# samuel-watson/glmmrMCML

Hardware: AMD Instinct MI355X
Metric: MCML iters/sec x m chains (simlik evals/sec) (higher is better)
Workload: dtype f64

## Files before the change

### glmmrmcml_amd/csrc/debug_hooks.hip

```cpp
#include "dgemm_mfma.h"
#include "dgemm_dl.h"
#include "dgemm_band.h"

using namespace mcml;

extern "C" int glmmr_mcml_dbg_dgemm(int M, int N, int K, const double* A, int lda,
                                    const double* B, int ldb, int b_nmajor,
                                    double alpha, double beta, double* C, int ldc,
                                    int lower_only, int force_tile)
{
    int ndev = 0;
    if (hipGetDeviceCount(&ndev) != hipSuccess || ndev == 0) {
        set_error("no HIP device: libglmmr_mcml_hip has no CPU fallback");
        return MCML_ENODEVICE;
    }
    hipStream_t s = nullptr;
    DevMat dA, dB, dC;
    if (force_tile == 40) {
        MCML_REQUIRE(!b_nmajor && !lower_only, "dbg_dgemm: the direct-to-LDS kernel takes a K-major B and all tiles");
        const int kpad = round_up(K, 32);
        MCML_TRY(dA.alloc(M, K, 32));
        MCML_HIP(hipMemset(dA.d(), 0, sizeof(double) * (size_t)dA.ld * dA.cols_alloc));
        MCML_HIP(hipMemcpy2D(dA.d(), sizeof(double) * dA.ld, A, sizeof(double) * lda, sizeof(double) * M, K, hipMemcpyHostToDevice));
        MCML_TRY(dB.alloc(kpad, N));
// ... 20 lines not shown
                      : launch_gemm<false>(s, M, N, K, dA.d(), dA.ld, dB.d(), dB.ld, epi, lower_only != 0, force_tile);
    MCML_TRY(rc);
    MCML_TRY(download_matrix(C, ldc, dC.d(), dC.ld, M, N, s));
    return MCML_OK;
}

extern "C" int glmmr_mcml_dbg_dgemm_at(int M, int N, int K, const double* A, int lda, const double* B, int ldb,
                                       double alpha, double beta, double* C, int ldc, int force_tile)
{
    int ndev = 0;
    if (hipGetDeviceCount(&ndev) != hipSuccess || ndev == 0) {
        set_error("no HIP device: libglmmr_mcml_hip has no CPU fallback");
        return MCML_ENODEVICE;
    }
    MCML_REQUIRE(M > 0 && N > 0 && K > 0 && A && B && C, "dbg_dgemm_at: bad argument");
    const int K2 = round_up(K, 2);
    MCML_REQUIRE(lda >= K2 && ldb >= K2 && ldc >= M, "dbg_dgemm_at: a column of A and of B holds round_up(K, 2) = %d doubles", K2);
    hipStream_t s = nullptr;
    DevMat dA, dB, dC;
    MCML_TRY(upload_matrix(dA, A, K2, M, lda, s));
    MCML_TRY(upload_matrix(dB, B, K2, N, ldb, s));
    const bool inplace = C == B;
    MCML_REQUIRE(!inplace || (M == K && M <= 128 && ldc == ldb), "dbg_dgemm_at: in place needs M == K <= 128");
    if (!inplace) MCML_TRY(upload_matrix(dC, C, M, N, ldc, s));
    const DevMat& out = inplace ? dB : dC;
    EpiAxpby epi{out.d(), out.ld, alpha, beta};
    MCML_TRY(launch_gemm_at(s, M, N, K, dA.d(), dA.ld, dB.d(), dB.ld, epi, force_tile));
    MCML_TRY(download_matrix(C, ldc, out.d(), out.ld, M, N, s));
    return MCML_OK;
}

extern "C" int glmmr_mcml_dbg_dgemm_bench2(int M, int N, int K, int b_nmajor, int iters, int force_tile,
                                           int lower_only, double beta, double* ms_per_launch);
extern "C" int glmmr_mcml_dbg_dgemm_bench(int M, int N, int K, int b_nmajor, int iters,
                                          int force_tile, double* ms_per_launch)
{
    return glmmr_mcml_dbg_dgemm_bench2(M, N, K, b_nmajor, iters, force_tile, 0, 0.0, ms_per_launch);
}

extern "C" int glmmr_mcml_dbg_dgemm_bench2(int M, int N, int K, int b_nmajor, int iters, int force_tile,
                                           int lower_only, double beta, double* ms_per_launch)
{
    int ndev = 0;
    if (hipGetDeviceCount(&ndev) != hipSuccess || ndev == 0) {
        set_error("no HIP device: libglmmr_mcml_hip has no CPU fallback");
        return MCML_ENODEVICE;
    }
    hipStream_t s = nullptr;
    std::vector<double> hA((size_t)M * K), hB((size_t)K * N), hC((size_t)M * N, 0.0);
    uint64_t x = 88172645463325252ULL;
    auto rnd = [&]() { x ^= x << 13; x ^= x >> 7; x ^= x << 17; return (double)(x >> 11) / 9007199254740992.0 * 2 - 1; };
    for (auto& v : hA) v = rnd();
    for (auto& v : hB) v = rnd();
    DevMat dA, dB, dC;
    MCML_TRY(upload_matrix(dA, hA.data(), M, K, M, s));
    if (b_nmajor) MCML_TRY(upload_matrix(dB, hB.data(), N, K, N, s));
    else MCML_TRY(upload_matrix(dB, hB.data(), K, N, K, s));
    MCML_TRY(upload_matrix(dC, hC.data(), M, N, M, s));
    EpiAxpby epi{dC.d(), dC.ld, beta != 0.0 ? 1e-3 : 1.0, beta};
    const bool lo = lower_only != 0;
    auto go = [&]() {
        if (force_tile >= 20)
            return b_nmajor ? launch_gemm_dl<true>(s, M, N, K, dA.d(), dA.ld, dB.d(), dB.ld, epi, lo, force_tile - 19)
                            : launch_gemm_dl<false>(s, M, N, K, dA.d(), dA.ld, dB.d(), dB.ld, epi, lo, force_tile - 19);
        return b_nmajor ? launch_gemm<true>(s, M, N, K, dA.d(), dA.ld, dB.d(), dB.ld, epi, lo, force_tile)
                        : launch_gemm<false>(s, M, N, K, dA.d(), dA.ld, dB.d(), dB.ld, epi, lo, force_tile);
    };
    for (int i = 0; i < 3; i++) MCML_TRY(go());
    hipEvent_t e0, e1;
    MCML_HIP(hipEventCreate(&e0));
    MCML_HIP(hipEventCreate(&e1));
    MCML_HIP(hipEventRecord(e0, s));
    for (int i = 0; i < iters; i++) MCML_TRY(go());
    MCML_HIP(hipEventRecord(e1, s));
    MCML_HIP(hipEventSynchronize(e1));
    float ms = 0;
    MCML_HIP(hipEventElapsedTime(&ms, e0, e1));
    *ms_per_launch = ms / iters;
    (void)hipEventDestroy(e0);
    (void)hipEventDestroy(e1);
    return MCML_OK;
}

extern "C" int glmmr_mcml_dbg_dgemm_band(int M, int N, int K, const double* A, int lda, const double* B, int ldb,
                                         double* C, int ldc, int* tiles_executed)
{
    int ndev = 0;
    if (hipGetDeviceCount(&ndev) != hipSuccess || ndev == 0) {
        set_error("no HIP device: libglmmr_mcml_hip has no CPU fallback");
        return MCML_ENODEVICE;
    }
    MCML_REQUIRE(M > 0 && N > 0 && K > 0 && A && B && C, "dbg_dgemm_band: bad argument");
    hipStream_t s = nullptr;
    DevMat dA, dB, dC;
    MCML_TRY(dA.alloc(M, K, 32));
    MCML_HIP(hipMemset(dA.d(), 0, sizeof(double) * (size_t)dA.ld * dA.cols_alloc));
    MCML_HIP(hipMemcpy2D(dA.d(), sizeof(double) * dA.ld, A, sizeof(double) * lda, sizeof(double) * M, K, hipMemcpyHostToDevice));
    MCML_TRY(dB.alloc(round_up(K, 32), N));
    MCML_HIP(hipMemset(dB.d(), 0, sizeof(double) * (size_t)dB.ld * N));
    MCML_HIP(hipMemcpy2D(dB.d(), sizeof(double) * dB.ld, B, sizeof(double) * ldb, sizeof(double) * K, N, hipMemcpyHostToDevice));
    MCML_TRY(dC.alloc(M, N));
    MCML_HIP(hipMemset(dC.d(), 0, sizeof(double) * (size_t)dC.ld * N));
    MCML_REQUIRE(dlds_applicable(M, N, K, dA.d(), dA.ld, dA.cols_alloc, dB.d(), dB.ld), "dbg_dgemm_band: contract");
    const int nbands = (M + BD_BM - 1) / BD_BM;
    DevBuf kr;
    MCML_TRY(kr.ensure(sizeof(int) * 2 * nbands));
    hipLaunchKernelGGL(k_band_ranges, dim3(nbands), dim3(256), 0, s, dA.d(), dA.ld, M, K, kr.as<int>());
    MCML_HIP(hipGetLastError());
    std::vector<int> hk(2 * nbands);
    MCML_HIP(hipMemcpy(hk.data(), kr.p, sizeof(int) * 2 * nbands, hipMemcpyDeviceToHost));
    BandPlan plan;
    plan.reset(M, K, hk);
    if (tiles_executed) *tiles_executed = (int)plan.tiles;
    EpiAxpby epi{dC.d(), dC.ld, 1.0, 0.0};
    MCML_TRY(launch_gemm_band(s, plan, N, dA.d(), dA.ld, dB.d(), dB.ld, epi));
    MCML_TRY(download_matrix(C, ldc, dC.d(), dC.ld, M, N, s));
    return MCML_OK;
}

extern "C" int glmmr_mcml_dbg_band_clocks(int M, int N, int iters, int mode, double* out3)
{
    int ndev = 0;
    if (hipGetDeviceCount(&ndev) != hipSuccess || ndev == 0) {
        set_error("no HIP device: libglmmr_mcml_hip has no CPU fallback");
        return MCML_ENODEVICE;
    }
    hipStream_t s = nullptr;
    if (getenv("GLMMR_MCML_DBG_STREAM")) MCML_HIP(hipStreamCreateWithFlags(&s, hipStreamNonBlocking));
    std::vector<double> hA((size_t)M * M, 0.0), hB((size_t)M * N);
    uint64_t x = 88172645463325252ULL;
    auto rnd = [&]() { x ^= x << 13; x ^= x >> 7; x ^= x << 17; return (double)(x >> 11) / 9007199254740992.0 * 2 - 1; };
    const bool cst = getenv("GLMMR_MCML_DBG_DATA") && !strcmp(getenv("GLMMR_MCML_DBG_DATA"), "const");
    const bool dec = getenv("GLMMR_MCML_DBG_DATA") && !strcmp(getenv("GLMMR_MCML_DBG_DATA"), "decay");
    for (int j = 0; j < M; ++j) for (int i = j; i < M; ++i) hA[i + (size_t)j * M] = cst ? 1.0 : dec ? rnd() * std::exp(-(double)(i - j) / 40.0) : rnd();
    for (auto& v : hB) v = cst ? 1.0 : rnd();
    DevMat dA, dB, dC;
    MCML_TRY(dA.alloc(M, M, 32));
    MCML_HIP(hipMemset(dA.d(), 0, sizeof(double) * (size_t)dA.ld * dA.cols_alloc));
    MCML_HIP(hipMemcpy2D(dA.d(), sizeof(double) * dA.ld, hA.data(), sizeof(double) * M, sizeof(double) * M, M, hipMemcpyHostToDevice));
    MCML_TRY(dB.alloc(round_up(M, 32), N));
    MCML_HIP(hipMemset(dB.d(), 0, sizeof(double) * (size_t)dB.ld * N));
    MCML_HIP(hipMemcpy2D(dB.d(), sizeof(double) * dB.ld, hB.data(), sizeof(double) * M, sizeof(double) * M, N, hipMemcpyHostToDevice));
    MCML_TRY(dC.alloc(M, N));
    const int nbands = (M + BD_BM - 1) / BD_BM;
    DevBuf kr, clk;
    MCML_TRY(kr.ensure(sizeof(int) * 2 * nbands));
    MCML_TRY(clk.ensure(16));
    MCML_HIP(hipMemset(clk.p, 0, 16));
    hipLaunchKernelGGL(k_band_ranges, dim3(nbands), dim3(256), 0, s, dA.d(), dA.ld, M, M, kr.as<int>());
    std::vector<int> hk(2 * nbands);
    MCML_HIP(hipMemcpy(hk.data(), kr.p, sizeof(int) * 2 * nbands, hipMemcpyDeviceToHost));
    BandPlan plan;
    plan.reset(M, M, hk);
    const double tiles = (double)plan.tiles;
    EpiAxpby epi{dC.d(), dC.ld, 1.0, 0.0};
    if (mode < 0) {
        for (int i = 0; i < 3; i++)
            MCML_TRY((launch_gemm_band<EpiAxpby, false>(s, plan, N, dA.d(), dA.ld, dB.d(), dB.ld, epi)));
        hipEvent_t f0, f1;
        MCML_HIP(hipEventCreate(&f0));
        MCML_HIP(hipEventCreate(&f1));
        MCML_HIP(hipEventRecord(f0, s));
        for (int i = 0; i < iters; i++)
            MCML_TRY((launch_gemm_band<EpiAxpby, false>(s, plan, N, dA.d(), dA.ld, dB.d(), dB.ld, epi)));
        MCML_HIP(hipEventRecord(f1, s));
        MCML_HIP(hipEventSynchronize(f1));
        float fms = 0;
        MCML_HIP(hipEventElapsedTime(&fms, f0, f1));
        out3[0] = fms / iters; out3[1] = 0;
        out3[2] = 2.0 * 80.0 * 32.0 * tiles * N / (fms / iters * 1e-3) / 1e12;
        (void)hipEventDestroy(f0);
        (void)hipEventDestroy(f1);
        return MCML_OK;
    }
    if (mode & 16) {
        BandPlanDev* d = nullptr;
        MCML_TRY(plan.device_plan((N + BD_BN - 1) / BD_BN, s, &d));
        const int nb = d->nwg * d->gn;
        DevBuf st;
        MCML_TRY(st.ensure(sizeof(unsigned long long) * (8 + 8 * (size_t)nb)));
        for (int rep = 0; rep < 3; ++rep) {
            MCML_HIP(hipMemset(st.p, 0, sizeof(unsigned long long) * (8 + 8 * (size_t)nb)));
            MCML_TRY((launch_gemm_band<EpiAxpby, true>(s, plan, N, dA.d(), dA.ld, dB.d(), dB.ld, epi, st.as<unsigned long long>(), mode)));
            MCML_HIP(hipDeviceSynchronize());
        }
        std::vector<unsigned long long> h(8 + 8 * (size_t)nb);
        MCML_HIP(hipMemcpy(h.data(), st.p, sizeof(unsigned long long) * h.size(), hipMemcpyDeviceToHost));
        unsigned long long t0 = ~0ULL;
        for (int w = 0; w < nb; ++w) if (h[8 + 8 * w] && h[8 + 8 * w] < t0) t0 = h[8 + 8 * w];
        double mx[5] = {0, 0, 0, 0, 0}, sm[5] = {0, 0, 0, 0, 0};
        for (int w = 0; w < nb; ++w)
            for (int i = 0; i < 5; ++i) { double v = (double)(h[8 + 8 * w + i] - t0) * 0.01; sm[i] += v; if (v > mx[i]) mx[i] = v; }
        printf("band stamps (us from the first workgroup's start; %d workgroups, mean / max):\n", nb);
        const char* nm[5] = {"start", "ring filled", "K loop done", "epilogue issued", "end"};
        for (int i = 0; i < 5; ++i) printf("  %-16s %7.2f / %7.2f\n", nm[i], sm[i] / nb, mx[i]);
        if (mode & 32) for (int w = 0; w < nb; ++w) {
            printf("  wg %3d:", w);
            for (int i = 0; i < 5; ++i) printf(" %7.2f", (double)(h[8 + 8 * w + i] - t0) * 0.01);
// ... 213 lines not shown
```

### glmmrmcml_amd/csrc/dgemm_band.h

```cpp
#pragma once
#include "dgemm_dlds.h"
#include "band_plan.h"

namespace mcml {

struct BandP {
    GemmP g;
    const BandItem* items;
    const int* wg_ptr;
    int nwg;
    double* part;
    int mode;
    unsigned long long* clocks;
};

static __global__ __launch_bounds__(256) void k_band_ranges(const double* A, int lda, int M, int K, int* krange)
{
    __shared__ int smin[256], smax[256];
    const int band = blockIdx.x, r0 = band * BD_BM;
    const int rows = (M - r0 < BD_BM) ? (M - r0) : BD_BM;
    int kmin = 1 << 30, kmax = -1;
    for (int k = threadIdx.x; k < K; k += 256) {
        const double* col = A + r0 + (size_t)k * lda;
        bool nz = false;
// ... 207 lines not shown
                const double* bs = reinterpret_cast<const double*>(lds + st * BD_STAGE_BYTES + BD_A_BYTES);
#pragma unroll
                for (int ks = 0; ks < BD_BK / 4; ++ks) {
                    const int kk = 4 * ks + lk;
                    double a[5];
#pragma unroll
                    for (int i = 0; i < 5; ++i) a[i] = as[kk * BD_BM + 16 * i + l15];
                    const double b = bs[((kk >> 1) * BD_BN + wave * 16 + l15) * 2 + (kk & 1)];
#pragma unroll
                    for (int i = 0; i < 5; ++i)
                        acc[i][0] = __builtin_amdgcn_mfma_f64_16x16x4f64(b, a[i], acc[i][0], 0, 0, 0);
                }
                wait_leave(issued - kt - 2);
                __builtin_amdgcn_s_barrier();
                st = st + 1; if (st >= BD_STAGES) st = 0;
            }
        } else if (DBG && nk > 0) {
            int issued = 0;
            if (!(mode & 1)) {
                for (; issued < BD_STAGES - 1 && issued < nk; ++issued) issue(issued);
                wait_leave(issued - 1);
            }
            __builtin_amdgcn_s_barrier();
            int st = 0;
            double a[5] = {1.0 + lane, 2.0, 3.0, 4.0, 5.0}, b = 0.5 + lane;
            for (int kt = 0; kt < nk; ++kt) {
                if (!(mode & 1) && issued < nk) {
                    int sn = st + BD_STAGES - 1; if (sn >= BD_STAGES) sn -= BD_STAGES;
                    issue(sn);
                    ++issued;
                }
                const double* as = reinterpret_cast<const double*>(lds + st * BD_STAGE_BYTES);
                const double* bs = reinterpret_cast<const double*>(lds + st * BD_STAGE_BYTES + BD_A_BYTES);
#pragma unroll
                for (int ks = 0; ks < BD_BK / 4; ++ks) {
                    const int kk = 4 * ks + lk;
                    if (!(mode & 4)) {
#pragma unroll
                        for (int i = 0; i < 5; ++i) a[i] = as[kk * BD_BM + 16 * i + l15];
                        b = bs[((kk >> 1) * BD_BN + wave * 16 + l15) * 2 + (kk & 1)];
                    }
#pragma unroll
                    for (int i = 0; i < 5; ++i)
                        acc[i][0] = __builtin_amdgcn_mfma_f64_16x16x4f64(b, a[i], acc[i][0], 0, 0, 0);
                }
                if (!(mode & 1)) wait_leave(issued - kt - 2);
                if (!(mode & 2)) __builtin_amdgcn_s_barrier();
                st = st + 1; if (st >= BD_STAGES) st = 0;
            }
        }
        if (first_item) stamp(2);
        ++it;
        pre = false;
        if (it < it1) {
            load_item(it);
            const int nkn = item.kt1 - item.kt0;
            if (mode == 0 && nk > 0 && nkn > 0) {
                issued = 0;
                for (; issued < BD_STAGES - 1 && issued < nkn; ++issued) issue(issued);
                pre = true;
            }
        }
        if (slot < 0) {
            epi(acc, e_m0, n0 + wave * 16, lane, p.M, p.N, band);
        } else {
            double* P = bp.part + ((size_t)slot * p.gn + bj) * BD_TILE_ELEMS + (size_t)wave * (20 * 64) + lane;
#pragma unroll
            for (int i = 0; i < 5; ++i)
#pragma unroll
                for (int r = 0; r < 4; ++r) P[(i * 4 + r) * 64] = acc[i][0][r];
        }
        if (first_item) { stamp(3); first_item = false; }
        if (!pre) __builtin_amdgcn_s_barrier();
    }
    if constexpr (DBG)
        if (stamps) { asm volatile("s_waitcnt vmcnt(0)" ::: "memory"); stamp(4); }
    if constexpr (DBG)
        if (bp.clocks && blockIdx.x == 0 && tid == 0) {
            atomicAdd(bp.clocks, __builtin_amdgcn_s_memtime() - t0c);
            atomicAdd(bp.clocks + 1, __builtin_amdgcn_s_memrealtime() - t0r);
        }
}

template <class Epi>
__global__ __launch_bounds__(128) void k_band_reduce(const BandRed* red, const double* part, int gn, int M, int N, Epi epi)
{
    const BandRed rd = red[blockIdx.x];
    const int bj = blockIdx.y;
    const int lane = threadIdx.x & 63, wave = blockIdx.z * 2 + (threadIdx.x >> 6);
    d4 acc[5][1];
#pragma unroll
    for (int i = 0; i < 5; ++i) acc[i][0] = d4{0.0, 0.0, 0.0, 0.0};
    const size_t pstride = (size_t)gn * BD_TILE_ELEMS;
    const double* P0 = part + ((size_t)rd.s0 * gn + bj) * BD_TILE_ELEMS + (size_t)wave * (20 * 64) + lane;
    for (int s = rd.s0; s < rd.s1; s += 4) {
        double v[4][20];
#pragma unroll
        for (int u = 0; u < 4; ++u) {
            const double* P = P0 + (size_t)(s - rd.s0 + (s + u < rd.s1 ? u : 0)) * pstride;
#pragma unroll
            for (int t = 0; t < 20; ++t) v[u][t] = P[t * 64];
        }
#pragma unroll
        for (int u = 0; u < 4; ++u)
            if (s + u < rd.s1) {
#pragma unroll
                for (int i = 0; i < 5; ++i)
#pragma unroll
                    for (int r = 0; r < 4; ++r) acc[i][0][r] += v[u][i * 4 + r];
            }
    }
    epi(acc, rd.band * BD_BM, bj * BD_BN + wave * 16, lane, M, N, rd.band);
}

template <class Epi, bool DBG = false>
static inline int launch_gemm_band(hipStream_t s, BandPlan& plan, int N, const double* A, int lda,
                                   const double* B, int ldb, const Epi& epi,
                                   unsigned long long* clocks = nullptr, int mode = 0)
{
    const int gn = (N + BD_BN - 1) / BD_BN;
    BandPlanDev* d = nullptr;
    MCML_TRY(plan.device_plan(gn, s, &d));
    BandP bp;
    bp.clocks = clocks;
    bp.mode = mode;
    bp.g = GemmP{plan.M, N, plan.K, A, lda, B, ldb, 0, gn, 0};
    bp.items = d->items.as<BandItem>();
    bp.wg_ptr = d->wg_ptr.as<int>();
    bp.nwg = d->nwg;
    bp.part = d->part.d();
    MCML_TRY(ensure_dynamic_lds(reinterpret_cast<const void*>(&dgemm_band_kernel<Epi, DBG>), (int)BD_LDS_BYTES));
    hipLaunchKernelGGL((dgemm_band_kernel<Epi, DBG>), dim3(d->nwg * gn), dim3(512), BD_LDS_BYTES, s, bp, epi);
    if (d->nred > 0)
        hipLaunchKernelGGL((k_band_reduce<Epi>), dim3(d->nred, gn, 4), dim3(128), 0, s, d->red.as<BandRed>(),
                           d->part.d(), gn, plan.M, N, epi);
    MCML_HIP(hipGetLastError());
    return MCML_OK;
}


}
```

### glmmrmcml_amd/csrc/hmc.hip

```cpp
#include <algorithm>
#include <atomic>
#include <chrono>
#include "../../include/glmmr_mcml_c.h"
#include "ctx.h"
#include "dgemm_mfma.h"
#include "dgemm_dlds.h"
#include "dgemm_band.h"
#include "dgemm_skinny.h"
#include "glm.h"
#include "reduce.h"
#include "rng.h"
#include "hmc_cm.h"
#include "hmc_traj.h"

namespace mcml {

struct ChainArrays {
    double *e, *ebar, *H, *lpcur, *K0;
    int *steps, *acc;
    uint32_t* gen;
    long long* leap;
};

static ChainArrays chain_arrays(const HmcState& h)
// ... 65 lines not shown
    const double* e; const int* steps; int s; double post; int mode;
    __device__ __forceinline__ void elem(int m, int n, double accv) const {
        int st = 0; double en = 0.0;
        if (mode == 1) { st = steps[n]; en = e[n]; if (s >= st) return; }
        const size_t off = m + (size_t)n * ld;
        const double x = Xs[off];
        double g = -1.0 * x;
        g = g + post * accv;
        if (mode != 1 || s + 1 >= st) G[off] = g;
        if (mode == 1) {
            double rr = R[off];
            rr = rr + (en / 2) * g;
            if (s + 1 < st) {
                rr = rr + (en / 2) * g;
                UP[off] = x + en * rr;
            }
            R[off] = rr;
        }
    }
    template <int TM, int TN>
    __device__ __forceinline__ void operator()(d4 (&acc)[TM][TN], int mB, int nB, int lane, int M, int N,
                                               int) const {
#pragma unroll
        for (int j = 0; j < TN; ++j) {
            int stv[4]; double env[4]; bool inN[4]; size_t cb[4];
#pragma unroll
            for (int r = 0; r < 4; ++r) {
                const int n = nB + 16 * j + (lane >> 4) + 4 * r;
                inN[r] = n < N;
                const int nn = inN[r] ? n : 0;
                stv[r] = mode == 1 ? steps[nn] : 0;
                env[r] = mode == 1 ? e[nn] : 0.0;
                cb[r] = (size_t)nn * ld;
            }
            double xv[TM][4], rv[TM][4];
#pragma unroll
            for (int i = 0; i < TM; ++i) {
                const int m = mB + 16 * i + (lane & 15);
                const int mm = m < M ? m : 0;
#pragma unroll
                for (int r = 0; r < 4; ++r) {
                    xv[i][r] = Xs[mm + cb[r]];
                    rv[i][r] = mode == 1 ? R[mm + cb[r]] : 0.0;
                }
            }
#pragma unroll
            for (int r = 0; r < 4; ++r) {
                const double en = env[r];
                const bool more = s + 1 < stv[r];
#pragma unroll
                for (int i = 0; i < TM; ++i) {
                    const double x = xv[i][r];
                    double g = -1.0 * x;
                    g = g + post * acc[i][j][r];
                    acc[i][j][r] = g;
                    double rr = rv[i][r];
                    rr = rr + (en / 2) * g;
                    const double rr2 = rr + (en / 2) * g;
                    rr = more ? rr2 : rr;
                    rv[i][r] = rr;
                    xv[i][r] = x + en * rr;
                }
            }
#pragma unroll
            for (int r = 0; r < 4; ++r) {
                const bool act = inN[r] && (mode != 1 || s < stv[r]);
                if (!act) continue;
                const bool more = s + 1 < stv[r];
#pragma unroll
                for (int i = 0; i < TM; ++i) {
                    const int m = mB + 16 * i + (lane & 15);
                    if (m >= M) continue;
                    const size_t off = m + cb[r];
                    if (mode != 1 || !more) G[off] = acc[i][j][r];
                    if (mode == 1) {
                        if (more) UP[off] = xv[i][r];
                        R[off] = rv[i][r];
                    }
                }
            }
        }
    }
};


__global__ __launch_bounds__(256) void k_blockdiag_LV(int Q, int ncols, const int* start, const double* L, int ldl,
                                                      const double* V, int ldv, double* U, int ldu)
{
    const int q = blockIdx.x * 256 + threadIdx.x;
    if (q >= Q) return;
    const int s0 = start[q];
    for (int c = blockIdx.y; c < ncols; c += gridDim.y) {
        const double* v = V + (size_t)c * ldv;
        double acc = 0.0;
        for (int t = s0; t <= q; ++t) acc += L[q + (size_t)t * ldl] * v[t];
        U[q + (size_t)c * ldu] = acc;
    }
}

__global__ __launch_bounds__(256) void k_hmc_init(double* V, int ld, int Q, ChainArrays ca, uint64_t seed,
                                                  uint32_t chain_offset, uint32_t iter_idx, const double* inj_init)
{
    const int c = blockIdx.x;
    const uint32_t gid = chain_offset + (uint32_t)c;
    for (int q = threadIdx.x; q < Q; q += 256)
        V[q + (size_t)c * ld] = inj_init ? inj_init[q + (size_t)c * Q]
                                         : rng_normal(seed, (uint32_t)q, gid, 0u, 16u * iter_idx + 0u);
    if (threadIdx.x == 0) {
        ca.e[c] = 0.001; ca.ebar[c] = 1.0; ca.H[c] = 0.0; ca.acc[c] = 0; ca.leap[c] = 0;
        ca.gen[c] = chain_minstd_seed(seed, gid, iter_idx);
        ca.steps[c] = 1;
    }
}

template <int FL>
__device__ __forceinline__ double chain_log_prob(const double* MU, int ldm, int n, const double* X, int ldx,
                                                 int Q, const double* y, double var_par, int flink_rt, int c,
                                                 double* sh)
{
    const int flink = FL ? FL : flink_rt;
    double ll = 0, lp = 0;
    for (int i0 = threadIdx.x; i0 < n; i0 += 1024) {
        double m4[4], y4[4];
#pragma unroll
        for (int u = 0; u < 4; ++u) {
            const int i = i0 + 256 * u;
            m4[u] = i < n ? MU[i + (size_t)c * ldm] : 0.0;
            y4[u] = i < n ? y[i] : 0.0;
        }
#pragma unroll
        for (int u = 0; u < 4; ++u)
            if (i0 + 256 * u < n) ll += glm_logpdf(y4[u], m4[u], var_par, flink);
    }
    for (int k0 = threadIdx.x; k0 < Q; k0 += 1024) {
        double x4[4];
#pragma unroll
        for (int u = 0; u < 4; ++u) { const int k = k0 + 256 * u; x4[u] = k < Q ? X[k + (size_t)c * ldx] : 0.0; }
#pragma unroll
        for (int u = 0; u < 4; ++u)
            if (k0 + 256 * u < Q) lp += glm_logpdf(x4[u], 0, 1, 7);
    }
    double a = block_sum(ll, sh);
    double b = block_sum(lp, sh);
    return a + b;
}

template <int FL>
__global__ __launch_bounds__(256) void k_hmc_lp0(const double* MU, int ldm, int n, const double* V, int ld, int Q,
                                                 const double* y, double var_par, int flink, double* lpcur)
{
    __shared__ double sh[4];
    double v = chain_log_prob<FL>(MU, ldm, n, V, ld, Q, y, var_par, flink, blockIdx.x, sh);
    if (threadIdx.x == 0) lpcur[blockIdx.x] = v;
}

__global__ __launch_bounds__(256) void k_hmc_propose(const double* V, const double* GRAD, double* R, double* UP,
                                                     int ld, int Q, ChainArrays ca, double lambda, int max_steps,
                                                     uint64_t seed, uint32_t chain_offset, uint32_t iter_idx,
                                                     int it, const double* inj_mom, int C)
{
    __shared__ double sh[4];
    const int c = blockIdx.x;
    const uint32_t gid = chain_offset + (uint32_t)c;
    const double e = ca.e[c];
    double ss = 0;
    for (int q = threadIdx.x; q < Q; q += 256) {
// ... 705 lines not shown
```

### include/glmmr_mcml_c.h

```cpp
#ifndef GLMMR_MCML_C_H
#define GLMMR_MCML_C_H
#include <stdint.h>

#ifdef __cplusplus
extern "C" {
#endif

#define GLMMR_MCML_OK            0
#define GLMMR_MCML_EINVAL       -1
#define GLMMR_MCML_EUNSUPPORTED -2
#define GLMMR_MCML_ENOTPD       -3
#define GLMMR_MCML_ESINGULAR    -4
#define GLMMR_MCML_EHIP         -5
#define GLMMR_MCML_ENODEVICE    -6
#define GLMMR_MCML_ENOMEM       -7

const char* glmmr_mcml_last_error(void);


typedef struct glmmr_mcml_problem {
    const int32_t* cov;
    int            cov_rows;
    const double*  data;
    int            data_len;
// ... 171 lines not shown
                     double* theta, double* sigma);
int glmmr_mcml_simlik(const glmmr_mcml_problem* prob, const double* u, int ucols, const double* start,
                      int nstart, int trace, const glmmr_mcml_ext* ext, double* beta, double* theta,
                      double* sigma);
int glmmr_mcml_optim_sparse(const glmmr_mcml_problem* prob, const int32_t* Ap, const int32_t* Ai, int nnz,
                            const double* u, int ucols, const double* start, int nstart, int trace,
                            int mcnr, const glmmr_mcml_ext* ext, double* beta, double* theta,
                            double* sigma,
                            int32_t* Lp, int32_t* Li, double* Lx, double* D, int lcap);
int glmmr_mcml_sparse_factor_nnz(const int32_t* cov, int cov_rows, const double* data, int data_len);
int glmmr_mcml_simlik_sparse(const glmmr_mcml_problem* prob, const int32_t* Ap, const int32_t* Ai, int nnz,
                             const double* u, int ucols, const double* start, int nstart, int trace,
                             const glmmr_mcml_ext* ext, double* beta, double* theta, double* sigma);
int glmmr_mcml_hess(const glmmr_mcml_problem* prob, const double* u, int ucols, const double* start,
                    int nstart, double tol, int trace, const glmmr_mcml_ext* ext, double* H);
int glmmr_mcml_hess_sparse(const glmmr_mcml_problem* prob, const int32_t* Ap, const int32_t* Ai, int nnz,
                           const double* u, int ucols, const double* start, int nstart, double tol,
                           int trace, const glmmr_mcml_ext* ext, double* H);
int glmmr_mcml_aic(const glmmr_mcml_problem* prob, const double* u, int ucols, const double* beta_par,
                   int nbeta, const double* cov_par, int ncov, const glmmr_mcml_ext* ext, double* out);

int glmmr_mcml_la(const glmmr_mcml_problem* prob, const double* start, int nstart, int usehess, double tol,
                  int verbose, int trace, int maxiter, const glmmr_mcml_ext* ext, double* beta, double* theta,
                  double* sigma, double* se, double* u);
int glmmr_mcml_la_nr(const glmmr_mcml_problem* prob, const double* start, int nstart, int usehess, double tol,
                     int verbose, int trace, int maxiter, const glmmr_mcml_ext* ext, double* beta, double* theta,
                     double* sigma, double* se, double* u);
int glmmr_mcml_ctx_la(glmmr_mcml_ctx* ctx, const double* start, int nstart, int nr, int usehess, double tol,
                      int verbose, int trace, int maxiter, const glmmr_mcml_ext* ext, double* beta, double* theta,
                      double* sigma, double* se, double* u, int* converged, int* iters);

int glmmr_mcml_mvn_ll(const int32_t* cov, int cov_rows, const double* data, int data_len,
                      const double* eff_range, int eff_len, const double* gamma, int ngamma,
                      const double* u, int Q, int m, double* out);

int glmmr_mcml_dbg_theta_log(glmmr_mcml_ctx* ctx, int enable, double* out, int cap_rows, int* nrows);
int glmmr_mcml_dbg_emulate_world(glmmr_mcml_ctx* ctx, int world, int mode);
int glmmr_mcml_dbg_leaf_profile(glmmr_mcml_ctx* ctx, unsigned long long* out10);
int glmmr_mcml_dbg_la_probe(glmmr_mcml_ctx* ctx, const double* start, int nstart, int kind, const double* v,
                            double var_par, const double* par, int npar, double* out, double* v_out,
                            double* beta_out, double* sigma_out);
int glmmr_mcml_dbg_dgemm(int M, int N, int K, const double* A, int lda, const double* B, int ldb,
                         int b_nmajor, double alpha, double beta, double* C, int ldc,
                         int lower_only, int force_tile );
int glmmr_mcml_dbg_dgemm_at(int M, int N, int K, const double* A, int lda, const double* B, int ldb, double alpha,
                            double beta, double* C, int ldc, int force_tile);
int glmmr_mcml_dbg_chol(glmmr_mcml_ctx* ctx, int n, double* A, int lda, int m, const double* B, int ldb, double* Xfwd,
                        double* Ytrans, double* Zpotrs, double* Linv);
int glmmr_mcml_dbg_mvn_workspace(glmmr_mcml_ctx* ctx, int cand, double* L, int ldl, double* X, int ldx, int* dims);
int glmmr_mcml_dbg_log_prob_grad(glmmr_mcml_ctx* ctx, const double* beta, double var_par, const double* V,
                                 int ncols, double* lp, double* G);
int glmmr_mcml_dbg_normals(uint64_t seed, uint32_t chain, uint32_t prop, uint32_t tag, int n, double* out);
int glmmr_mcml_dbg_minstd(uint32_t seed, int n, double* out);
typedef double (*glmmr_mcml_objective)(const double* x, int n, void* user);
int glmmr_mcml_dbg_bobyqa(glmmr_mcml_objective f, void* user, int n, const double* x0, const double* lower,
                          const double* upper, double rhobeg, double rhoend, int maxfun, double* x_out,
                          double* f_out, int* nfev_out);
int glmmr_mcml_dbg_bobyqa_npt(glmmr_mcml_objective f, void* user, int n, const double* x0, const double* lower,
                              const double* upper, double rhobeg, double rhoend, int maxfun, int npt, double* x_out,
                              double* f_out, int* nfev_out);
int glmmr_mcml_dbg_bobyqa_batch(glmmr_mcml_objective f, void* user, int n, const double* x0, const double* lower,
                                const double* upper, double rhobeg, double rhoend, int maxfun, int width,
                                double* x_out, double* f_out, int* nfev_out, int* rounds_out);
typedef int (*glmmr_mcml_batch_objective)(const double* X, int n, int k, double* F, void* user);
int glmmr_mcml_dbg_bobyqa_rounds(glmmr_mcml_batch_objective fb, void* user, int n, const double* x0, const double* lower,
                                 const double* upper, double rhobeg, double rhoend, int maxfun, int width,
                                 double* x_out, double* f_out, int* nfev_out, int* rounds_out);
typedef int (*glmmr_mcml_parts_objective)(const double* X, int n, int k, double* logdet, double* sumsq, int* status,
                                          void* user);
int glmmr_mcml_dbg_theta_scale_rounds(glmmr_mcml_parts_objective fb, void* user, int n, const int* exps, int dim, int m,
                                      int grouped, const double* x0, const double* lower, const double* upper,
                                      double rhobeg, double rhoend, int maxfun, int width, double* x_out, double* f_out,
                                      int* nfev_out, int* rounds_out, long long* factorised_out);
int glmmr_mcml_dbg_theta_round(glmmr_mcml_ctx* ctx, const double* thetas, int k, double* out);
int glmmr_mcml_dbg_copy_roundtrip(const double* in, long long ld_in, double* out, long long ld_out, long long rows, long long cols);
int glmmr_mcml_dbg_fd_hessian(glmmr_mcml_objective f, void* user, int n, const double* x, double ndeps,
                              int usebounds, const double* lower, const double* upper, double* H);
int glmmr_mcml_dbg_dgemm_bench(int M, int N, int K, int b_nmajor, int iters, int force_tile,
                               double* ms_per_launch);
int glmmr_mcml_dbg_dgemm_bench2(int M, int N, int K, int b_nmajor, int iters, int force_tile, int lower_only,
                                double beta, double* ms_per_launch);
int glmmr_mcml_dbg_dgemm_band(int M, int N, int K, const double* A, int lda, const double* B, int ldb, double* C,
                              int ldc, int* tiles_executed);
int glmmr_mcml_dbg_band_clocks(int M, int N, int iters, int mode, double* out3);

#ifdef __cplusplus
}
#endif
#endif
```

Measured before the change: 1161.

## Add warp-specialised feeder form of band DGEMM with dedicated DMA waves

Adds a new band GEMM kernel in which four waves only issue global-to-LDS DMA loads through a multi-stage buffer. The other four waves only run f64 MFMA work on a 32-column slice each, with double-buffered LDS register reads. It is enabled by default, overridable through an env var, for the axpby and HMC forward/backward epilogues. The aim is to keep load issue and waitcnt stalls off the MFMA waves. The cost is half the waves doing no math and larger per-wave accumulators.

New measurement: 1223 (median of 6 runs). 5.3% higher.

```diff
diff --git a/glmmrmcml_amd/csrc/debug_hooks.hip b/glmmrmcml_amd/csrc/debug_hooks.hip
--- a/glmmrmcml_amd/csrc/debug_hooks.hip
+++ b/glmmrmcml_amd/csrc/debug_hooks.hip
@@ -126,8 +126,24 @@
     return MCML_OK;
 }
 
+static int dbg_dgemm_band(int M, int N, int K, const double* A, int lda, const double* B, int ldb, double* C, int ldc,
+                          int* tiles_executed, int form, int* whole_band);
+
 extern "C" int glmmr_mcml_dbg_dgemm_band(int M, int N, int K, const double* A, int lda, const double* B, int ldb,
                                          double* C, int ldc, int* tiles_executed)
+{
+    return dbg_dgemm_band(M, N, K, A, lda, B, ldb, C, ldc, tiles_executed, BAND_FORM_AUTO, nullptr);
+}
+
+extern "C" int glmmr_mcml_dbg_dgemm_band_form(int M, int N, int K, const double* A, int lda, const double* B, int ldb,
+                                              double* C, int ldc, int* tiles_executed, int form, int* whole_band)
+{
+    MCML_REQUIRE(form == BAND_FORM_8WAVE || form == BAND_FORM_FEED, "dbg_dgemm_band_form: form is 0 or 1");
+    return dbg_dgemm_band(M, N, K, A, lda, B, ldb, C, ldc, tiles_executed, form, whole_band);
+}
+
+static int dbg_dgemm_band(int M, int N, int K, const double* A, int lda, const double* B, int ldb, double* C, int ldc,
+                          int* tiles_executed, int form, int* whole_band)
 {
     int ndev = 0;
     if (hipGetDeviceCount(&ndev) != hipSuccess || ndev == 0) {
@@ -157,7 +173,7 @@
     plan.reset(M, K, hk);
     if (tiles_executed) *tiles_executed = (int)plan.tiles;
     EpiAxpby epi{dC.d(), dC.ld, 1.0, 0.0};
-    MCML_TRY(launch_gemm_band(s, plan, N, dA.d(), dA.ld, dB.d(), dB.ld, epi));
+    MCML_TRY(launch_gemm_band(s, plan, N, dA.d(), dA.ld, dB.d(), dB.ld, epi, nullptr, 0, form, whole_band));
     MCML_TRY(download_matrix(C, ldc, dC.d(), dC.ld, M, N, s));
     return MCML_OK;
 }
diff --git a/glmmrmcml_amd/csrc/dgemm_band.h b/glmmrmcml_amd/csrc/dgemm_band.h
--- a/glmmrmcml_amd/csrc/dgemm_band.h
+++ b/glmmrmcml_amd/csrc/dgemm_band.h
@@ -313,6 +313,222 @@
         }
 }
 
+template <class Epi> struct BandFeed { static constexpr bool ok = false; };
+template <> struct BandFeed<EpiAxpby> { static constexpr bool ok = true; };
+
+constexpr int BF_NA = 5, BF_NB = 8, BF_PER_TILE = BF_NA + BF_NB;
+static_assert(4 * BF_NA * 1024 == BD_A_BYTES && 4 * BF_NB * 1024 == BD_B_BYTES, "four feeders cover a stage");
+
+static inline bool band_feed_enabled()
+{
+    const char* e = getenv("GLMMR_MCML_BAND_FEED");
+    return !(e && !strcmp(e, "0"));
+}
+
+template <int KS>
+__device__ __forceinline__ void bf_read(double (&a)[5], double (&b)[2], unsigned aaddr, unsigned baddr)
+{
+    BD_RD(a[0], aaddr, KS * 4 * BD_BM * 8);
+    BD_RD(a[1], aaddr, KS * 4 * BD_BM * 8 + 128);
+    BD_RD(a[2], aaddr, KS * 4 * BD_BM * 8 + 256);
+    BD_RD(a[3], aaddr, KS * 4 * BD_BM * 8 + 384);
+    BD_RD(a[4], aaddr, KS * 4 * BD_BM * 8 + 512);
+    BD_RD(b[0], baddr, KS * 2 * BD_BN * 16);
+    BD_RD(b[1], baddr, KS * 2 * BD_BN * 16 + 256);
+}
+template <int LEAVE>
+__device__ __forceinline__ void bf_wait(double (&a)[5], double (&b)[2])
+{
+#if defined(__HIP_DEVICE_COMPILE__)
+    if constexpr (LEAVE == 7)
+        asm volatile("s_waitcnt lgkmcnt(7)" : "+v"(a[0]), "+v"(a[1]), "+v"(a[2]), "+v"(a[3]), "+v"(a[4]), "+v"(b[0]), "+v"(b[1]));
+    else
+        asm volatile("s_waitcnt lgkmcnt(0)" : "+v"(a[0]), "+v"(a[1]), "+v"(a[2]), "+v"(a[3]), "+v"(a[4]), "+v"(b[0]), "+v"(b[1]));
+#endif
+}
+__device__ __forceinline__ void bf_mfma(d4 (&acc)[2][5][1], const double (&a)[5], const double (&b)[2])
+{
+#pragma unroll
+    for (int j = 0; j < 2; ++j)
+#pragma unroll
+        for (int i = 0; i < 5; ++i) acc[j][i][0] = __builtin_amdgcn_mfma_f64_16x16x4f64(b[j], a[i], acc[j][i][0], 0, 0, 0);
+}
+__device__ __forceinline__ BandItem bf_item(const BandItem* ip)
+{
+    BandItem item{0, 0, 0, -1};
+#if defined(__HIP_DEVICE_COMPILE__)
+    typedef int i4s __attribute__((ext_vector_type(4)));
+    i4s raw;
+    asm volatile("s_load_dwordx4 %0, %1, 0x0\n\ts_waitcnt lgkmcnt(0)" : "=&s"(raw) : "s"(ip) : "memory");
+    item.band = raw.x; item.kt0 = raw.y; item.kt1 = raw.z; item.slot = raw.w;
+#else
+    item = *ip;
+#endif
+    return item;
+}
+
+template <class Epi>
+__global__ __launch_bounds__(512) void dgemm_band_feed_kernel(BandP bp, Epi epi)
+{
+    const GemmP& p = bp.g;
+    extern __shared__ __attribute__((aligned(16))) double smem[];
+    char* lds = reinterpret_cast<char*>(smem);
+    const int tid = threadIdx.x, lane = tid & 63, wave = __builtin_amdgcn_readfirstlane(tid >> 6);
+    const unsigned lds0 = (unsigned)(size_t)(lds_ptr_t)lds;
+
+    const int nblk = bp.nwg * p.gn;
+    const int bid = blockIdx.x;
+    const int q8 = nblk >> 3, r8 = nblk & 7, xcd = bid & 7;
+    const int nid = (xcd < r8 ? xcd * (q8 + 1) : r8 * (q8 + 1) + (xcd - r8) * q8) + (bid >> 3);
+    const int pw = nid / p.gn, bj = nid - pw * p.gn;
+    const int n0 = bj * BD_BN;
+    const int it0 = bp.wg_ptr[pw], it1 = bp.wg_ptr[pw + 1];
+
+    if (wave >= 4) {
+        const int f = wave - 4;
+        const size_t stepA = (size_t)BD_BK * p.lda * 8;
+        unsigned vob[BF_NB];
+#pragma unroll
+        for (int s = 0; s < BF_NB; ++s) {
+            const int c = f + 4 * s;
+            const int kp = c >> 1, n = ((c & 1) << 6) + lane;
+            int gn = n0 + n;
+            if (gn >= p.N) gn = 0;
+            vob[s] = (unsigned)((2 * kp + (size_t)gn * p.ldb) * 8);
+        }
+        unsigned voa[BF_NA];
+        const char* sA = nullptr; const char* sB = nullptr;
+        BandItem item{0, 0, 0, -1};
+        auto load_item = [&](int it) {
+            item = bf_item(bp.items + it);
+            const int m0 = item.band * BD_BM;
+#pragma unroll
+            for (int s = 0; s < BF_NA; ++s) {
+                const int o = (f + 4 * s) * 1024 + lane * 16;
+                const int k = o / (BD_BM * 8), m = (o - k * BD_BM * 8) >> 3;
+                int gm = m0 + m;
+                if (gm >= p.M) gm = 0;
+                voa[s] = (unsigned)((gm + (size_t)k * p.lda) * 8);
+            }
+            sA = reinterpret_cast<const char*>(p.A) + (size_t)item.kt0 * stepA;
+            sB = reinterpret_cast<const char*>(p.B) + (size_t)item.kt0 * (BD_BK * 8);
+        };
+        auto issue = [&](int stage) {
+            const unsigned lbase = lds0 + stage * BD_STAGE_BYTES + f * 1024;
+#pragma unroll
+            for (int s = 0; s < BF_NA; ++s) lds_dma16(lbase + s * 4096, voa[s], sA);
+#pragma unroll
+            for (int s = 0; s < BF_NB; ++s) lds_dma16(lbase + BD_A_BYTES + s * 4096, vob[s], sB);
+            sA += stepA;
+            sB += BD_BK * 8;
+        };
+        auto wait_leave = [&](int tiles) {
+            static_assert(BF_PER_TILE == 13, "vmcnt immediates below");
+            if (tiles >= 2) asm volatile("s_waitcnt vmcnt(26)" ::: "memory");
+            else if (tiles == 1) asm volatile("s_waitcnt vmcnt(13)" ::: "memory");
+            else asm volatile("s_waitcnt vmcnt(0)" ::: "memory");
+        };
+        bool pre = false;
+        int issued = 0;
+        if (it0 < it1) load_item(it0);
+        for (int it = it0; it < it1;) {
+            const int nk = item.kt1 - item.kt0;
+            if (nk > 0) {
+                if (!pre) { issued = 0; for (; issued < BD_STAGES - 1 && issued < nk; ++issued) issue(issued); }
+                wait_leave(issued - 1);
+                __builtin_amdgcn_s_barrier();
+                int st = 0;
+                for (int kt = 0; kt < nk; ++kt) {
+                    if (issued < nk) {
+                        int sn = st + BD_STAGES - 1; if (sn >= BD_STAGES) sn -= BD_STAGES;
+                        issue(sn);
+                        ++issued;
+                    }
+                    wait_leave(issued - kt - 2);
+                    __builtin_amdgcn_s_barrier();
+                    ++st; if (st >= BD_STAGES) st = 0;
+                }
+            }
+            ++it;
+            pre = false;
+            if (it < it1) {
+                load_item(it);
+                const int nkn = item.kt1 - item.kt0;
+                if (nk > 0 && nkn > 0) {
+                    issued = 0;
+                    for (; issued < BD_STAGES - 1 && issued < nkn; ++issued) issue(issued);
+                    pre = true;
+                }
+            }
+            if (!pre) __builtin_amdgcn_s_barrier();
+        }
+        return;
+    }
+
+    const int l15 = lane & 15, lk = lane >> 4;
+    const unsigned aoff = lds0 + lk * (BD_BM * 8) + l15 * 8;
+    const unsigned boff = lds0 + BD_A_BYTES + (((lk >> 1) * BD_BN + wave * 32 + l15) << 4) + ((lk & 1) << 3);
+    BandItem item{0, 0, 0, -1};
+    if (it0 < it1) item = bf_item(bp.items + it0);
+    for (int it = it0; it < it1;) {
+        const int band = item.band, e_m0 = item.band * BD_BM, slot = item.slot;
+        const int nk = item.kt1 - item.kt0;
+
+        d4 acc[2][5][1];
+#pragma unroll
+        for (int j = 0; j < 2; ++j)
+#pragma unroll
+            for (int i = 0; i < 5; ++i) acc[j][i][0] = d4{0.0, 0.0, 0.0, 0.0};
+
+        if (nk > 0) {
+            __builtin_amdgcn_s_barrier();
+            int st = 0;
+            double ra[2][5], rb[2][2];
+            bf_read<0>(ra[0], rb[0], aoff, boff);
+            for (int kt = 0; kt < nk; ++kt) {
+                const unsigned aaddr = aoff + st * BD_STAGE_BYTES, baddr = boff + st * BD_STAGE_BYTES;
+                int stn = st + 1; if (stn >= BD_STAGES) stn = 0;
+#define BF_STEP(KS, CUR, NXT)                                   \
+                bf_read<KS + 1>(ra[NXT], rb[NXT], aaddr, baddr); \
+                bf_wait<7>(ra[CUR], rb[CUR]);                    \
+                bf_mfma(acc, ra[CUR], rb[CUR]);                  \
+                __builtin_amdgcn_sched_barrier(0);
+                BF_STEP(0, 0, 1) BF_STEP(1, 1, 0) BF_STEP(2, 0, 1) BF_STEP(3, 1, 0)
+                BF_STEP(4, 0, 1) BF_STEP(5, 1, 0) BF_STEP(6, 0, 1)
+#undef BF_STEP
+                bf_wait<0>(ra[1], rb[1]);
+                __builtin_amdgcn_s_barrier();
+                if (kt + 1 < nk) bf_read<0>(ra[0], rb[0], aoff + stn * BD_STAGE_BYTES, boff + stn * BD_STAGE_BYTES);
+                bf_mfma(acc, ra[1], rb[1]);
+                __builtin_amdgcn_sched_barrier(0);
+                st = stn;
+            }
+        }
+        ++it;
+        bool pre = false;
+        if (it < it1) {
+            item = bf_item(bp.items + it);
+            pre = nk > 0 && item.kt1 - item.kt0 > 0;
+        }
+        if (slot < 0) {
+            int elane = lane;
+            asm volatile("" : "+v"(elane));
+            epi(acc[0], e_m0, n0 + wave * 32, elane, p.M, p.N, band);
+            __builtin_amdgcn_sched_barrier(0);
+            epi(acc[1], e_m0, n0 + wave * 32 + 16, elane, p.M, p.N, band);
+        } else {
+            double* P = bp.part + ((size_t)slot * p.gn + bj) * BD_TILE_ELEMS + (size_t)(2 * wave) * (20 * 64) + lane;
+#pragma unroll
+            for (int j = 0; j < 2; ++j)
+#pragma unroll
+                for (int i = 0; i < 5; ++i)
+#pragma unroll
+                    for (int r = 0; r < 4; ++r) P[(j * 20 + i * 4 + r) * 64] = acc[j][i][0][r];
+        }
+        if (!pre) __builtin_amdgcn_s_barrier();
+    }
+}
+
 template <class Epi>
 __global__ __launch_bounds__(128) void k_band_reduce(const BandRed* red, const double* part, int gn, int M, int N, Epi epi)
 {
@@ -344,10 +560,12 @@
     epi(acc, rd.band * BD_BM, bj * BD_BN + wave * 16, lane, M, N, rd.band);
 }
 
+enum { BAND_FORM_AUTO = -1, BAND_FORM_8WAVE = 0, BAND_FORM_FEED = 1 };
 template <class Epi, bool DBG = false>
 static inline int launch_gemm_band(hipStream_t s, BandPlan& plan, int N, const double* A, int lda,
                                    const double* B, int ldb, const Epi& epi,
-                                   unsigned long long* clocks = nullptr, int mode = 0)
+                                   unsigned long long* clocks = nullptr, int mode = 0, int form = BAND_FORM_AUTO,
+                                   int* whole_band = nullptr)
 {
     const int gn = (N + BD_BN - 1) / BD_BN;
     BandPlanDev* d = nullptr;
@@ -360,8 +578,20 @@
     bp.wg_ptr = d->wg_ptr.as<int>();
     bp.nwg = d->nwg;
     bp.part = d->part.d();
-    MCML_TRY(ensure_dynamic_lds(reinterpret_cast<const void*>(&dgemm_band_kernel<Epi, DBG>), (int)BD_LDS_BYTES));
-    hipLaunchKernelGGL((dgemm_band_kernel<Epi, DBG>), dim3(d->nwg * gn), dim3(512), BD_LDS_BYTES, s, bp, epi);
+    if (whole_band) *whole_band = d->paired;
+    bool feed = false;
+    if constexpr (BandFeed<Epi>::ok && !DBG) {
+        feed = form == BAND_FORM_AUTO ? band_feed_enabled() : form == BAND_FORM_FEED;
+        if (feed) {
+            MCML_TRY(ensure_dynamic_lds(reinterpret_cast<const void*>(&dgemm_band_feed_kernel<Epi>), (int)BD_LDS_BYTES));
+            hipLaunchKernelGGL((dgemm_band_feed_kernel<Epi>), dim3(d->nwg * gn), dim3(512), BD_LDS_BYTES, s, bp, epi);
+        }
+    }
+    MCML_REQUIRE(feed || form != BAND_FORM_FEED, "launch_gemm_band: no feeder form of this instantiation");
+    if (!feed) {
+        MCML_TRY(ensure_dynamic_lds(reinterpret_cast<const void*>(&dgemm_band_kernel<Epi, DBG>), (int)BD_LDS_BYTES));
+        hipLaunchKernelGGL((dgemm_band_kernel<Epi, DBG>), dim3(d->nwg * gn), dim3(512), BD_LDS_BYTES, s, bp, epi);
+    }
     if (d->nred > 0)
         hipLaunchKernelGGL((k_band_reduce<Epi>), dim3(d->nred, gn, 4), dim3(128), 0, s, d->red.as<BandRed>(),
                            d->part.d(), gn, plan.M, N, epi);
diff --git a/glmmrmcml_amd/csrc/hmc.hip b/glmmrmcml_amd/csrc/hmc.hip
--- a/glmmrmcml_amd/csrc/hmc.hip
+++ b/glmmrmcml_amd/csrc/hmc.hip
@@ -171,6 +171,11 @@
         }
     }
 };
+
+template <> struct BandFeed<EpiBackward> { static constexpr bool ok = true; };
+template <> struct BandFeed<EpiForwardT<1>> { static constexpr bool ok = true; };
+template <> struct BandFeed<EpiForwardT<3>> { static constexpr bool ok = true; };
+template <> struct BandFeed<EpiForwardT<7>> { static constexpr bool ok = true; };
 
 
 __global__ __launch_bounds__(256) void k_blockdiag_LV(int Q, int ncols, const int* start, const double* L, int ldl,
diff --git a/include/glmmr_mcml_c.h b/include/glmmr_mcml_c.h
--- a/include/glmmr_mcml_c.h
+++ b/include/glmmr_mcml_c.h
@@ -277,6 +277,8 @@
                                 double beta, double* ms_per_launch);
 int glmmr_mcml_dbg_dgemm_band(int M, int N, int K, const double* A, int lda, const double* B, int ldb, double* C,
                               int ldc, int* tiles_executed);
+int glmmr_mcml_dbg_dgemm_band_form(int M, int N, int K, const double* A, int lda, const double* B, int ldb, double* C,
+                                   int ldc, int* tiles_executed, int form, int* whole_band);
 int glmmr_mcml_dbg_band_clocks(int M, int N, int iters, int mode, double* out3);
 
 #ifdef __cplusplus
```
